# eezkni/UEGAN

Hardware: AMD Instinct MI355X
Metric: train imgs/sec @512px bs=16 on 1/2/4/8 MI355X; infer ms/img (higher is better)
Workload: dtype bf16; 1 GPU; FiveK-shaped 512x512 batch=16/GPU, full G/D/VGG train step (trainer.py:77-119), conv_dim=32, seeded stand-in VGG19; global_batch=16, parallelism=dp1, pool_size=50, collective=none (1 rank), passes=batched (fused.py)

## Files before the change

### include/uegan_hip.h

```cpp
#ifndef UEGAN_HIP_H_
#define UEGAN_HIP_H_

#include <stddef.h>
#include <stdint.h>

#ifdef __cplusplus
extern "C" {
#endif

#define UEGAN_VERSION 105

enum { UEGAN_OK = 0, UEGAN_E_INVALID = -1, UEGAN_E_HIP = -2, UEGAN_E_UNSUPPORTED = -3 };
enum { UEGAN_F32 = 0, UEGAN_BF16 = 1 };
enum { UEGAN_PAD_ZERO = 0, UEGAN_PAD_REFLECT = 1 };
enum { UEGAN_ACT_NONE = 0, UEGAN_ACT_LRELU = 1, UEGAN_ACT_RELU = 2, UEGAN_ACT_TANH = 3,
       UEGAN_ACT_SIGMOID = 4,
       UEGAN_ACT_SWISH = 5, UEGAN_ACT_SELU = 6 };
enum { UEGAN_IMPL_AUTO = 0, UEGAN_IMPL_MFMA = 1, UEGAN_IMPL_DIRECT = 2, UEGAN_IMPL_MFMA_REGSTAGE = 3, UEGAN_IMPL_MFMA_GENERIC = 4 };

typedef void* uegan_stream_t;

int uegan_version(void);
const char* uegan_last_error(void);
int uegan_set_conv_impl(int impl);
enum {
  UEGAN_TUNE_SMALL_GRID = 0,
  UEGAN_TUNE_FOLD_MAX = 1,
  UEGAN_TUNE_HEADS_NO_CG = 2,
  UEGAN_TUNE_WIDE_MIN_GRID = 3,
  UEGAN_TUNE_TALL_MIN_GRID = 4,
  UEGAN_TUNE_TALL_RPW = 5,
  UEGAN_TUNE_TALL_REFLECT = 6,
  UEGAN_TUNE_FLAT_S2 = 7,
  UEGAN_TUNE_TOEP_HEADS = 8,
  UEGAN_TUNE_HEADS_MFMA = 9,
  UEGAN_TUNE_FWD_STATS = 10,
  UEGAN_TUNE_WGRAD_XCD = 11,
  UEGAN_TUNE_VGG_EPI = 12,
  UEGAN_TUNE_GAM_BWD = 13,
  UEGAN_TUNE_COUNT = 14
};
int uegan_set_tuning(int knob, int value, int* previous);
int uegan_selftest_mfma(void* scratch_4096_floats, uegan_stream_t stream);

typedef struct {
  char name[96];
  int64_t launches;
  double total_ms;
  double total_flops;
  double total_bytes;
} uegan_profile_entry;
int uegan_profile_begin(int max_records);
int uegan_profile_end(uegan_profile_entry* out, int max_entries, int* n_entries);

typedef struct {
  int32_t dtype;
  int32_t B, H, W;
  int32_t C1, C2;
  int32_t Ho, Wo, Cout;
  int32_t KH, KW, stride, pad;
  int32_t pad_mode;
  int32_t act;
  int32_t Cin_w, Cout_w;
  int32_t Cin_total;
  int32_t scale_group;
} uegan_conv_desc;

int64_t uegan_packed_k(int64_t k);
int uegan_pack_weights(int dtype, const float* w_oihw, int Cout, int Cin, int KH, int KW, int Cout_pad, int Cin_pad, void* w_ohwi,
                       void* w_ihwo, uegan_stream_t stream);
int uegan_pack_weights_slice(int dtype, const float* w_oihw, int Cout, int Cin, int Cin_total, int KH, int KW, int Cout_pad, int Cin_pad,
                             void* w_ohwi, void* w_ihwo, uegan_stream_t stream);
int uegan_pack_weights_pair(int dtype, const float* w_oihw, int Cout, int Cin, int Cin_total, int KH, int KW, int Cout_pad, int Cin_pad,
                            void* w_ohwi, void* w_ihwo, void* w_ohwi_lo, int dup_cin, uegan_stream_t stream);
typedef struct uegan_pack_entry {
  const float* w_oihw;
  void* w_ohwi;
  void* w_ihwo;
  int64_t start;
  int32_t Cout, Cin, Cin_total, KH, KW, Cout_pad, Cin_pad, Kp, Kp2;
  int32_t flags;
  void* w_ohwi_lo;
} uegan_pack_entry;
int uegan_pack_weights_multi(int dtype, const uegan_pack_entry* table_dev, int n_entries, int64_t total, uegan_stream_t stream);
int uegan_conv2d_fwd(const uegan_conv_desc* d, const void* x1, const void* x2, const void* w_ohwi, const float* bias,
                     const float* scale, void* y, uegan_stream_t stream);
size_t uegan_conv2d_fwd_splitk_workspace_bytes(const uegan_conv_desc* d);
int uegan_conv2d_fwd_splitk(const uegan_conv_desc* d, const void* x1, const void* x2, const void* w_ohwi, const float* bias, const float* scale, void* y,
                            void* workspace, size_t workspace_bytes, uegan_stream_t stream);
size_t uegan_conv2d_fwd_stats_workspace_bytes(const uegan_conv_desc* d);
int uegan_conv2d_fwd_stats(const uegan_conv_desc* d, const void* x1, const void* x2, const void* w_ohwi, const float* bias, const float* scale, void* y,
                           float* mean, float* rstd, float eps, void* workspace, size_t workspace_bytes, int* produced, uegan_stream_t stream);
int uegan_instnorm_apply(int dtype, const void* x, void* y, const float* mean, const float* rstd, int B, int HW, int C, uegan_stream_t stream);
// ... 280 lines not shown
```

### uegan_amd/csrc/conv.hip

```cpp
#include "conv_stream.h"

namespace uegan {

int check_desc(const uegan_conv_desc* d) {
  UEGAN_CHECK_ARG(d != nullptr, "conv desc is null");
  UEGAN_CHECK_ARG(d->dtype == UEGAN_F32 || d->dtype == UEGAN_BF16, "bad dtype %d", d->dtype);
  UEGAN_CHECK_ARG(d->B > 0 && d->H > 0 && d->W > 0 && d->C1 > 0 && d->C2 >= 0 && d->Cout > 0, "bad conv dims");
  UEGAN_CHECK_ARG(d->KH > 0 && d->KW > 0 && d->stride > 0 && d->pad >= 0, "bad conv kernel/stride/pad");
  UEGAN_CHECK_ARG(d->Ho == (d->H + 2 * d->pad - d->KH) / d->stride + 1 && d->Wo == (d->W + 2 * d->pad - d->KW) / d->stride + 1,
                  "Ho/Wo inconsistent with H,W,pad,K,stride");
  if (d->pad_mode == UEGAN_PAD_REFLECT)
    UEGAN_CHECK_ARG(d->pad < d->H && d->pad < d->W, "reflection pad %d must be smaller than the input (%d x %d)", d->pad, d->H, d->W);
  else
    UEGAN_CHECK_ARG(d->pad_mode == UEGAN_PAD_ZERO, "bad pad mode");
  const int epc = d->dtype == UEGAN_F32 ? 4 : 8;
  UEGAN_CHECK_ARG(d->C1 % epc == 0 && d->C2 % epc == 0 && d->Cout % epc == 0,
                  "tensor channel counts must be multiples of %d (one 16-byte chunk): pad them (C1=%d C2=%d Cout=%d)", epc, d->C1, d->C2, d->Cout);
  UEGAN_CHECK_ARG(d->Cin_w >= 0 && d->Cin_w <= d->C1 + d->C2 && d->Cout_w >= 0 && d->Cout_w <= d->Cout, "bad true weight dims");
  UEGAN_CHECK_ARG(d->stride <= 2, "stride > 2 is not built");
  UEGAN_CHECK_ARG(d->scale_group >= 0, "bad scale_group");
  UEGAN_CHECK_ARG(d->Cin_total == 0 || d->Cin_total >= (d->Cin_w ? d->Cin_w : d->C1 + d->C2), "Cin_total must cover the input channels used");
  return UEGAN_OK;
}

ConvGeom fwd_geom(const uegan_conv_desc* d) {
  ConvGeom g;
  g.B = d->B; g.IH = d->H; g.IW = d->W; g.C1 = d->C1; g.C2 = d->C2; g.C = d->C1 + d->C2;
  g.OH = d->Ho; g.OW = d->Wo; g.KH = d->KH; g.KW = d->KW; g.stride = d->stride; g.pad = d->pad; g.pad_mode = d->pad_mode;
  g.mode = 0;
  return g;
}

}

using namespace uegan;

static size_t esize(int dtype) { return dtype == UEGAN_F32 ? 4 : 2; }
static int report_taken(int rc, int* flag, int value) {
  if (rc == UEGAN_OK) *flag = value;
  return rc == 1 ? UEGAN_OK : rc;
}

static void fwd_args(const uegan_conv_desc* d, ConvArgs& a, const void* x1, const void* x2, const void* w_ohwi, const float* bias, const float* scale, void* y) {
  a.g = fwd_geom(d);
  a.in1 = x1; a.in2 = d->C2 ? x2 : x1; a.w = w_ohwi; a.bias = bias; a.scale = scale; a.scale_group = d->scale_group; a.out = y; a.out2 = nullptr; a.n_out1 = 0;
  a.N = d->Cout; a.nbias = cout_w(d); a.Kp = (int)uegan_packed_k((int64_t)d->KH * d->KW * a.g.C); a.act = d->act;
  a.frame = 0; a.fy0 = a.fy1 = a.fx0 = a.fx1 = 0; a.mask = nullptr; a.mask_act = UEGAN_ACT_NONE;
}
static void dgrad_args(const uegan_conv_desc* d, ConvArgs& a, const void* dz, const void* w_ihwo, const float* scale, void* out1, void* out2, bool padded_grid) {
  ConvGeom& g = a.g;
  const int grow = padded_grid ? 2 * d->pad : 0;
  g.B = d->B; g.IH = d->Ho; g.IW = d->Wo; g.C1 = d->Cout; g.C2 = 0; g.C = d->Cout;
  g.OH = d->H + grow; g.OW = d->W + grow; g.KH = d->KH; g.KW = d->KW; g.stride = d->stride;
  g.pad = padded_grid ? 0 : d->pad; g.pad_mode = padded_grid ? UEGAN_PAD_ZERO : d->pad_mode;
  g.mode = 1;
  a.in1 = dz; a.in2 = dz; a.bias = nullptr; a.nbias = 0; a.scale = scale; a.scale_group = d->scale_group; a.act = UEGAN_ACT_NONE;
  a.Kp = (int)uegan_packed_k((int64_t)d->KH * d->KW * d->Cout);
  a.w = w_ihwo; a.N = d->C1 + d->C2;
  a.out = out1; a.out2 = d->C2 ? out2 : nullptr; a.n_out1 = d->C1;
  a.frame = 0; a.fy0 = a.fy1 = a.fx0 = a.fx1 = 0; a.mask = nullptr; a.mask_act = UEGAN_ACT_NONE;
}
static size_t padded_grid_bytes(const uegan_conv_desc* d) {
  return (size_t)d->B * (d->H + 2 * d->pad) * (d->W + 2 * d->pad) * (d->C1 + d->C2) * esize(d->dtype);
}

enum GatherRoute { ROUTE_DIRECT, ROUTE_TOEP, ROUTE_STREAM, ROUTE_MFMA };
static GatherRoute gather_route(const ConvArgs& a, int dtype, ConvStreamPlan& sp) {
  if (g_impl.impl == UEGAN_IMPL_DIRECT) return ROUTE_DIRECT;
  if (g_impl.glds && g_impl.stream && conv_toep_takes(a, dtype)) return ROUTE_TOEP;
  if (g_impl.glds && conv_stream_plan(a, dtype, sp)) return ROUTE_STREAM;
  return ROUTE_MFMA;
}
static bool patch_family(const ConvGeom& g, int dtype) { return g_impl.patch && g_impl.glds && g.KH == g.KW && g.C % (CONV_ROWB / (int)esize(dtype)) == 0; }
static int patch_ks(const ConvGeom& g, int dtype) {
  if (!patch_family(g, dtype)) return 0;
  if (g.stride == 1) {
    if (g.KH == 1 && g.pad == 0) return 1;
    if (g.KH == 3 || g.KH == 5 || g.KH == 7) return g.KH;
  } else if (g.stride == 2 && g.mode == 1) {
    if (g.KH == 3 || g.KH == 5 || g.KH == 7) return (g.KH + 1) / 2;
  }
  return 0;
}
static bool wide_first(const ConvGeom& g, int dtype) { return g.stride == 1 && patch_ks(g, dtype) == 3; }

static bool fwd_on_heads(const uegan_conv_desc* d) { return g_impl.impl != UEGAN_IMPL_DIRECT && g_impl.heads && heads_applicable(d); }
static bool dgrad_on_heads(const uegan_conv_desc* d) { return g_impl.impl != UEGAN_IMPL_DIRECT && g_impl.heads && heads_dgrad_applicable(d); }

static int patch_run(ConvArgs& a, int dtype, hipStream_t s, int ks) {
  if (dtype == UEGAN_F32) return ks <= 3 ? conv_patch_f32_a(a, s, ks) : conv_patch_f32_b(a, s, ks);
  return ks <= 3 ? conv_patch_bf16_a(a, s, ks) : conv_patch_bf16_b(a, s, ks);
}

static int dispatch_conv_gemm(ConvArgs& a, int dtype, hipStream_t s) {
  const ConvGeom& g = a.g;
  if (g_impl.patch && g_impl.glds && g.KH == g.KW && g.stride == 2 && g.mode == 0 && dtype != UEGAN_F32 && g.C == 32) {
    const int rc = conv_s2fwd_run(a, dtype, s);
    if (rc != 1) return rc;
  }
  if (patch_family(g, dtype)) {
    if (wide_first(g, dtype)) {
      int rc = conv_tall_run(a, dtype, s);
      if (rc != 1) return rc;
      rc = conv_wide_run(a, dtype, s);
      if (rc != 1) return rc;
      rc = conv_interior_run(a, dtype, s);
      if (rc != 1 && rc != UEGAN_OK) return rc;
    }
    const int ks = patch_ks(g, dtype);
    if (ks) return patch_run(a, dtype, s, ks);
    const int rc = conv_s2fwd_run(a, dtype, s);
    if (rc != 1) return rc;
  }
  return conv_gemm_run(a, dtype, s);
}

static int run_gather_gemm(ConvArgs& a, int dtype, hipStream_t s, bool* mask_applied = nullptr) {
  if (mask_applied) *mask_applied = false;
  ConvStreamPlan sp;
  switch (gather_route(a, dtype, sp)) {
    case ROUTE_DIRECT: return conv_gemm_run(a, dtype, s);
    case ROUTE_TOEP: return conv_toep_run(a, dtype, s);
    case ROUTE_STREAM:
      if (mask_applied) *mask_applied = a.mask != nullptr;
      {
        ProfScope prof = conv_stream_prof(sp, a.g.mode, s);
        conv_stream_launch(sp, s);
        UEGAN_CHECK_LAUNCH();
      }
      return sp.fixup ? launch_dgrad_images(a, dtype, s, sp.a.xmir != 0) : UEGAN_OK;
    case ROUTE_MFMA: break;
  }
  const int ks = a.g.stride == 1 ? patch_ks(a.g, dtype) : 0;
  if (!(a.g.mode == 1 && ((ks == 3 && a.g.pad_mode != UEGAN_PAD_REFLECT) || ks == 1))) a.mask = nullptr;
  if (mask_applied) *mask_applied = a.mask != nullptr;
  return dispatch_conv_gemm(a, dtype, s);
}

extern "C" int uegan_conv2d_fwd(const uegan_conv_desc* d, const void* x1, const void* x2, const void* w_ohwi, const float* bias,
                                const float* scale, void* y, uegan_stream_t stream) {
  int rc = check_desc(d);
  if (rc) return rc;
  UEGAN_CHECK_ARG(x1 && w_ohwi && y && (d->C2 == 0 || x2), "null pointer");
  ConvArgs a;
  fwd_args(d, a, x1, x2, w_ohwi, bias, scale, y);
  hipStream_t s = (hipStream_t)stream;
  if (fwd_on_heads(d)) {
    ConvStreamPlan sp;
    if (d->act == UEGAN_ACT_SIGMOID || gather_route(a, d->dtype, sp) == ROUTE_MFMA) return heads_fwd(d, x1, w_ohwi, bias, scale, y, s);
  }
// ... 367 lines not shown
```

### uegan_amd/csrc/conv_wide.hip

```cpp
#include "conv_core.h"

namespace uegan {

static __device__ __attribute__((aligned(128))) const unsigned int g_zero_page[512] = {0u};

typedef float f32x16 __attribute__((ext_vector_type(16)));

__device__ __forceinline__ f32x16 mfma32_bf16(u32x4 a, u32x4 b, f32x16 c) {
#ifdef UEGAN_HALF_FP16
  return __builtin_amdgcn_mfma_f32_32x32x16_f16(__builtin_bit_cast(bf16x8_t, a), __builtin_bit_cast(bf16x8_t, b), c, 0, 0, 0);
#else
  return __builtin_amdgcn_mfma_f32_32x32x16_bf16(__builtin_bit_cast(bf16x8_t, a), __builtin_bit_cast(bf16x8_t, b), c, 0, 0, 0);
#endif
}

#define UEGAN_SB() __builtin_amdgcn_sched_barrier(0)

template <int KS, int MODE, bool MASK, int ABL = 0>
__global__ void __launch_bounds__(256, 1) conv_wide_kernel(ConvArgs a) {
  constexpr int TH = 8, TW = 32, BN = 256, NWAVES = 4;
  constexpr int PH = TH + KS - 1, PW = TW + KS - 1;
  constexpr int NPG = (PH * PW + 7) / 8;
  constexpr int NI_P = (NPG + NWAVES - 1) / NWAVES;
  constexpr int PBUFB = NPG * 1024, WHALF = BN * 64, DUMPB = 4096;
// ... 200 lines not shown
    for (int i = 0; i < 4; ++i) {
      f32x4 bv[4];
#pragma unroll
      for (int q = 0; q < 4; ++q) bv[q] = *reinterpret_cast<const f32x4*>(lds_bias + (wn * 128 + i * 32 + 4 * lh + 8 * q) * 4);
#pragma unroll
      for (int j = 0; j < 4; ++j) {
        unsigned char* row = est + (j * 32 + l31) * EROW + i * 64 + 8 * lh;
#pragma unroll
        for (int q = 0; q < 4; ++q) {
          float v[4];
#pragma unroll
          for (int r = 0; r < 4; ++r) {
            const float z = plain ? acc[i][j][4 * q + r] : acc[i][j][4 * q + r] * scale + bv[q][r];
            v[r] = plain ? z : fmaxf(z, slope * z);
          }
          u32x2 pk;
          pk.x = pack_bf16x2(v[0], v[1]);
          pk.y = pack_bf16x2(v[2], v[3]);
          *reinterpret_cast<u32x2*>(row + q * 16) = pk;
        }
      }
    }
  }
  __builtin_amdgcn_wave_barrier();
  {
    const float mslope = a.mask_act == UEGAN_ACT_LRELU ? 0.2f : (a.mask_act == UEGAN_ACT_RELU ? 0.f : 1.f);
    bf16_t* out = static_cast<bf16_t*>(a.out);
    const int nl = n0 + wn * 128 + (lane & 15) * 8;
#pragma unroll 4
    for (int it = 0; it < 32; ++it) {
      const int rr = it * 4 + (lane >> 4);
      const int oy = y0 + wm * 4 + (rr >> 5), ox = x0 + (rr & 31);
      const u32x2 v01 = *reinterpret_cast<const u32x2*>(est + rr * EROW + (lane & 15) * 16);
      const u32x2 v23 = *reinterpret_cast<const u32x2*>(est + rr * EROW + (lane & 15) * 16 + 8);
      u32x4 v = {v01.x, v01.y, v23.x, v23.y};
      if (oy >= g.OH || ox >= g.OW) continue;
      const size_t pix = ((size_t)b * g.OH + oy) * g.OW + ox;
      const size_t o = pix * a.N + nl;
      if (MASK) {
        const u32x4 m = *reinterpret_cast<const u32x4*>(static_cast<const bf16_t*>(a.mask) + o);
#pragma unroll
        for (int d = 0; d < 4; ++d) {
          const float lo = half_lo_to_f32(v[d]) * (half_lo_to_f32(m[d]) > 0.f ? 1.f : mslope);
          const float hi = half_hi_to_f32(v[d]) * (half_hi_to_f32(m[d]) > 0.f ? 1.f : mslope);
          v[d] = pack_bf16x2(lo, hi);
        }
      }
      bf16_t* dst = !a.out2 ? out + o : (nl < a.n_out1 ? out + pix * a.n_out1 + nl : static_cast<bf16_t*>(a.out2) + pix * (a.N - a.n_out1) + (nl - a.n_out1));
      *reinterpret_cast<u32x4*>(dst) = v;
    }
  }
}

template <int NI, int MODE, bool MASK, bool POOL, int RPW = 4, int EPI = 0>
__global__ void __launch_bounds__(256, RPW == 2 ? 2 : 1) conv_tall_kernel(ConvArgs a) {
  static_assert(RPW == 4 || RPW == 2, "rows per wave");
  constexpr bool REFL = MODE == 2;
  static_assert(!REFL || (NI == 4 && !MASK && !POOL), "mirrored images: 128-channel blocks, plain epilogue");
  static_assert(EPI == 0 || (MODE == 1 && MASK && !POOL), "fidelity-loss epilogues: masked data gradients");
  constexpr int KS = 3, TH = 4 * RPW, TW = 32, BN = NI * 32, NWAVES = 4;
  constexpr int PH = TH + KS - 1, PW = TW + KS - 1, NPIX = PH * PW;
  constexpr int NPG = (NPIX + 15) / 16;
  constexpr int NI_P = (NPG + NWAVES - 1) / NWAVES;
  constexpr int PBUFB = NPG * 1024, WSL = BN * 64, NWP = WSL / 1024 / NWAVES;
  constexpr int DUMPB = RPW == 2 ? 1024 : 4096, DUMPW = RPW == 2 ? 0 : 1024;
  constexpr int NT = KS * KS, NLOAD = NWP + 2;
  constexpr bool DGRAD = MODE != 0;
  constexpr int EROW = BN * 2 + 8;
  constexpr int WPIX = RPW * 32;
  constexpr int MAINB = 2 * PBUFB + 4 * WSL, EPIB = NWAVES * WPIX * EROW;
  constexpr int BODYB = MAINB > EPIB ? MAINB : EPIB;
  static_assert(NI_P <= 2 * (NT - 2), "the next chunk's patch pieces must be requested two steps before the chunk ends");
  static_assert((RPW == 2 ? 2 : 1) * (BODYB + DUMPB + BN * 4) <= 160 * 1024, "LDS budget");
  static_assert(NWP >= 1, "at least one weight piece per wave per slice");

  __shared__ __attribute__((aligned(16))) unsigned char lds[BODYB + DUMPB + BN * 4];
  unsigned char* const lds_w = lds + 2 * PBUFB;
  unsigned char* const lds_dump = lds + BODYB;
  unsigned char* const lds_bias = lds_dump + DUMPB;

  const ConvGeom& g = a.g;
  const bf16_t* in1 = static_cast<const bf16_t*>(a.in1);
  const bf16_t* in2 = static_cast<const bf16_t*>(a.in2);
  const bf16_t* w = static_cast<const bf16_t*>(a.w);
  const int tid = threadIdx.x, lane = tid & 63;
  const int wave = __builtin_amdgcn_readfirstlane(tid >> 6);
  const int l31 = lane & 31, lh = lane >> 5;
  int n0 = blockIdx.y * BN;
  int t = blockIdx.x;
  if (a.xcd_map) {
    const int L = blockIdx.x + gridDim.x * blockIdx.y, nby = gridDim.y;
    const int xcd = L & 7, grp = L >> 3;
    n0 = (grp % nby) * BN;
    t = (grp / nby) * 8 + xcd;
  }
  const int tile_x = t % a.ntx; t /= a.ntx;
  const int tile_y = t % a.nty;
  const int b = t / a.nty;
  const int y0 = a.rect_y0 + tile_y * TH, x0 = a.rect_x0 + tile_x * TW;
  const int nchunk = g.C / 32, nchunk1 = g.C1 / 32;
  const int nsteps = nchunk * NT;

  const int q_src = ((lane & 3) ^ ((lane >> 4) & 3)) * 8;
  int ppix[NI_P];
  {
    const int vy0 = DGRAD ? y0 + g.pad - (KS - 1) : y0 - g.pad;
    const int vx0 = DGRAD ? x0 + g.pad - (KS - 1) : x0 - g.pad;
    const bool refl = !DGRAD && g.pad_mode == UEGAN_PAD_REFLECT;
#pragma unroll
    for (int ii = 0; ii < NI_P; ++ii) {
      const int pr = (ii * NWAVES + wave) * 16 + (lane >> 2);
      int pix = -1;
      if (pr < NPIX) {
        const int piy = pr / PW, pix_x = pr - piy * PW;
        int sy = vy0 + piy, sx = vx0 + pix_x;
        if (refl) { sy = reflect_idx(sy, g.IH); sx = reflect_idx(sx, g.IW); }
        if (sy >= 0 && sy < g.IH && sx >= 0 && sx < g.IW) pix = (b * g.IH + sy) * g.IW + sx;
      }
      ppix[ii] = pix;
    }
  }
  const unsigned char* const zero16 = reinterpret_cast<const unsigned char*>(g_zero_page) + (lane & 3) * 16;
  const unsigned char* p_src = zero16;
// ... 42 lines not shown
    if constexpr (REFL) xpr[j] = pr;
  };
  bool r_top[RPW], r_bot[RPW];
  bool e_left = false, e_right = false, c_left = false, c_right = false, edge = false;
  if constexpr (REFL) {
#pragma unroll
    for (int j = 0; j < RPW; ++j) {
      const int y = y0 + wave * RPW + j;
      r_top[j] = y == 1;
      r_bot[j] = y == g.OH - 2;
      edge = edge || r_top[j] || r_bot[j];
    }
    e_left = x0 == 0;
    e_right = x0 <= g.OW - 2 && g.OW - 2 < x0 + TW;
    c_left = x0 + l31 == 1;
    c_right = x0 + l31 == g.OW - 2;
    edge = edge || e_left || e_right;
  } else {
#pragma unroll
    for (int j = 0; j < RPW; ++j) r_top[j] = r_bot[j] = false;
  }
  auto fold1 = [&](u32x4& F, const unsigned char* pb, int ksub, int j, int tap) {
    const int ty = tap / KS, tx = tap - ty * KS;
    const bool ym = ty == 0 ? r_top[j] : (ty == 2 ? r_bot[j] : false);
    const bool xany = tx == 0 ? e_left : (tx == 2 ? e_right : false);
    if (!ym && !xany) return;
    const int dpy = ty == 0 ? -2 * PW : 2 * PW, dpx = tx == 0 ? -2 : 2;
    auto rd = [&](int pr) { return *reinterpret_cast<const u32x4*>(pb + ((pr * 64 + ((lh ^ ((pr >> 2) & 3)) << 4)) ^ (ksub << 5))); };
    if (ym) F = add_frag<bf16_t>(F, rd(xpr[j] + dpy));
    if (xany) {
      const uint32_t m = (tx == 0 ? c_left : c_right) ? 0xffffffffu : 0u;
      u32x4 v = rd(xpr[j] + dpx);
      if (ym) v = add_frag<bf16_t>(v, rd(xpr[j] + dpy + dpx));
      F = add_frag<bf16_t>(F, v & u32x4{m, m, m, m});
    }
  };
  u32x4 wf0[NI], xf0[RPW], wf1[NI], xf1[RPW];
  f32x16 acc[NI][RPW];
#pragma unroll
  for (int i = 0; i < NI; ++i)
#pragma unroll
    for (int j = 0; j < RPW; ++j)
#pragma unroll
      for (int r = 0; r < 16; ++r) acc[i][j][r] = 0.f;
  const bool plain = !a.scale && !a.bias && a.act == UEGAN_ACT_NONE;
  {
    const int n = n0 + wave * 64 + lane;
    const bool live = wave * 64 < BN && !plain && a.bias && n < a.nbias;
    __builtin_amdgcn_global_load_lds((const __attribute__((address_space(1))) void*)(live ? a.bias + n : reinterpret_cast<const float*>(g_zero_page) + lane),
                                     (__attribute__((address_space(3))) void*)(wave * 64 < BN ? lds_bias + wave * 256 : lds_dump + wave * DUMPW), 4, 0, 0);
  }
  const float scale = a.scale ? a.scale[a.scale_group ? b / a.scale_group : 0] : 1.f;

#pragma unroll
  for (int ii = 0; ii < NI_P; ++ii) { patch_piece_prepare(ii, 0, true); patch_piece_issue(); }
#pragma unroll
  for (int h = 0; h < 3; ++h) {
    stage_w_prepare();
#pragma unroll
    for (int i = 0; i < NWP; ++i) stage_w_piece(i);
  }
  wait_vmcnt<NWP>();
  raw_barrier();
#pragma unroll
  for (int j = 0; j < RPW; ++j) set_xad(0, j);
#pragma unroll
  for (int i = 0; i < NI; ++i) wf0[i] = *reinterpret_cast<const u32x4*>(lds_w + wad[i]);
#pragma unroll
  for (int j = 0; j < RPW; ++j) xf0[j] = *reinterpret_cast<const u32x4*>(lds + xad[j]);

#define MF(W, X, i, j) acc[i][j] = mfma32_bf16(W[i], X[j], acc[i][j]); UEGAN_SB();
#define LDW(F, slot, ksub, i) F[i] = *reinterpret_cast<const u32x4*>((slot) + (wad[i] ^ ((ksub) << 5)));
#define LDX(F, pb, ksub, j) F[j] = *reinterpret_cast<const u32x4*>((pb) + (xad[j] ^ ((ksub) << 5)));
#define FOLDX(F, pb, ksub, tapv)                                                           \
  if constexpr (REFL) {                                                                    \
    if (edge) {                                                                            \
      _Pragma("unroll") for (int jf = 0; jf < RPW; ++jf) fold1(F[jf], pb, ksub, jf, tapv); \
    }                                                                                      \
  }
  FOLDX(xf0, lds, 0, 0)
  for (int chunk = 0; chunk < nchunk; ++chunk) {
    const unsigned char* pcur = lds + (chunk & 1) * PBUFB;
    const bool more = chunk + 1 < nchunk;
#pragma unroll
    for (int tap = 0; tap < NT; ++tap) {
      const int step = chunk * NT + tap;
      const unsigned char* ws = lds_w + (step & 3) * WSL;
      const unsigned char* wnext = lds_w + ((step + 1) & 3) * WSL;
      const unsigned char* pnext = tap + 1 == NT ? lds + ((chunk + 1) & 1) * PBUFB : pcur;
      const int ntap = tap + 1 == NT ? 0 : tap + 1;
      UEGAN_SB();
      if constexpr (RPW == 2 && NI == 2) {
        MF(wf0, xf0, 0, 0) LDW(wf1, ws, 1, 0) LDW(wf1, ws, 1, 1) UEGAN_SB();
        MF(wf0, xf0, 0, 1) LDX(xf1, pcur, 1, 0) LDX(xf1, pcur, 1, 1) UEGAN_SB();
        MF(wf0, xf0, 1, 0) stage_w_prepare(); stage_w_piece(0); UEGAN_SB();
        if (2 * tap < NI_P) {
          MF(wf0, xf0, 1, 1) patch_piece_prepare(2 * tap, chunk + 1, more); patch_piece_issue(); patch_piece_prepare(2 * tap + 1, chunk + 1, more); patch_piece_issue(); UEGAN_SB();
        } else {
          MF(wf0, xf0, 1, 1)
        }
        MF(wf1, xf1, 0, 0) set_xad(ntap, 0); set_xad(ntap, 1); UEGAN_SB();
        MF(wf1, xf1, 0, 1) LDW(wf0, wnext, 0, 0) LDW(wf0, wnext, 0, 1) UEGAN_SB();
        MF(wf1, xf1, 1, 0) LDX(xf0, pnext, 0, 0) LDX(xf0, pnext, 0, 1) UEGAN_SB();
        MF(wf1, xf1, 1, 1)
      } else if constexpr (RPW == 2) {
        MF(wf0, xf0, 0, 0) LDW(wf1, ws, 1, 0) LDW(wf1, ws, 1, 1) UEGAN_SB();
// ... 11 lines not shown
        MF(wf1, xf1, 1, 1) LDX(xf0, pnext, 0, 0) LDX(xf0, pnext, 0, 1) UEGAN_SB();
        MF(wf1, xf1, 2, 0) MF(wf1, xf1, 2, 1) MF(wf1, xf1, 3, 0) MF(wf1, xf1, 3, 1)
        FOLDX(xf0, pnext, 0, ntap)
      } else if constexpr (NI == 4) {
        MF(wf0, xf0, 0, 0) stage_w_prepare(); UEGAN_SB();
        MF(wf0, xf0, 0, 1) stage_w_piece(0); UEGAN_SB();
        MF(wf0, xf0, 0, 2) stage_w_piece(1); UEGAN_SB();
        MF(wf0, xf0, 0, 3) patch_piece_prepare(2 * tap, chunk + 1, more); UEGAN_SB();
        MF(wf0, xf0, 1, 0) patch_piece_issue(); UEGAN_SB();
        MF(wf0, xf0, 1, 1) patch_piece_prepare(2 * tap + 1, chunk + 1, more); UEGAN_SB();
        MF(wf0, xf0, 1, 2) patch_piece_issue(); UEGAN_SB();
        MF(wf0, xf0, 1, 3) LDW(wf1, ws, 1, 0) LDW(wf1, ws, 1, 1) UEGAN_SB();
        MF(wf0, xf0, 2, 0) LDW(wf1, ws, 1, 2) LDW(wf1, ws, 1, 3) UEGAN_SB();
        MF(wf0, xf0, 2, 1) LDX(xf1, pcur, 1, 0) LDX(xf1, pcur, 1, 1) UEGAN_SB();
        MF(wf0, xf0, 2, 2) LDX(xf1, pcur, 1, 2) LDX(xf1, pcur, 1, 3) UEGAN_SB();
        MF(wf0, xf0, 2, 3) MF(wf0, xf0, 3, 0) MF(wf0, xf0, 3, 1) MF(wf0, xf0, 3, 2) MF(wf0, xf0, 3, 3)
        FOLDX(xf1, pcur, 1, tap)
        MF(wf1, xf1, 0, 0) set_xad(ntap, 0); UEGAN_SB();
        MF(wf1, xf1, 0, 1) set_xad(ntap, 1); UEGAN_SB();
        MF(wf1, xf1, 0, 2) set_xad(ntap, 2); UEGAN_SB();
        MF(wf1, xf1, 0, 3) set_xad(ntap, 3); UEGAN_SB();
        MF(wf1, xf1, 1, 0) LDW(wf0, wnext, 0, 0) LDW(wf0, wnext, 0, 1) UEGAN_SB();
        MF(wf1, xf1, 1, 1) LDW(wf0, wnext, 0, 2) LDW(wf0, wnext, 0, 3) UEGAN_SB();
        MF(wf1, xf1, 1, 2) LDX(xf0, pnext, 0, 0) LDX(xf0, pnext, 0, 1) UEGAN_SB();
        MF(wf1, xf1, 1, 3) LDX(xf0, pnext, 0, 2) LDX(xf0, pnext, 0, 3) UEGAN_SB();
        MF(wf1, xf1, 2, 0) MF(wf1, xf1, 2, 1) MF(wf1, xf1, 2, 2) MF(wf1, xf1, 2, 3)
        MF(wf1, xf1, 3, 0) MF(wf1, xf1, 3, 1) MF(wf1, xf1, 3, 2) MF(wf1, xf1, 3, 3)
        FOLDX(xf0, pnext, 0, ntap)
      } else {
        static_assert(NI == 2 || NI == 4, "channel fragments per wave");
        MF(wf0, xf0, 0, 0) LDW(wf1, ws, 1, 0) LDW(wf1, ws, 1, 1) UEGAN_SB();
        MF(wf0, xf0, 0, 1) LDX(xf1, pcur, 1, 0) LDX(xf1, pcur, 1, 1) UEGAN_SB();
        MF(wf0, xf0, 0, 2) LDX(xf1, pcur, 1, 2) LDX(xf1, pcur, 1, 3) UEGAN_SB();
        MF(wf0, xf0, 0, 3) stage_w_prepare(); UEGAN_SB();
        MF(wf0, xf0, 1, 0) stage_w_piece(0); UEGAN_SB();
        MF(wf0, xf0, 1, 1) patch_piece_prepare(2 * tap, chunk + 1, more); UEGAN_SB();
        MF(wf0, xf0, 1, 2) patch_piece_issue(); patch_piece_prepare(2 * tap + 1, chunk + 1, more); UEGAN_SB();
        MF(wf0, xf0, 1, 3) patch_piece_issue(); UEGAN_SB();
        MF(wf1, xf1, 0, 0) set_xad(ntap, 0); set_xad(ntap, 1); UEGAN_SB();
        MF(wf1, xf1, 0, 1) set_xad(ntap, 2); set_xad(ntap, 3); LDW(wf0, wnext, 0, 0) LDW(wf0, wnext, 0, 1) UEGAN_SB();
        MF(wf1, xf1, 0, 2) LDX(xf0, pnext, 0, 0) LDX(xf0, pnext, 0, 1) UEGAN_SB();
        MF(wf1, xf1, 0, 3) LDX(xf0, pnext, 0, 2) LDX(xf0, pnext, 0, 3) UEGAN_SB();
        MF(wf1, xf1, 1, 0) MF(wf1, xf1, 1, 1) MF(wf1, xf1, 1, 2) MF(wf1, xf1, 1, 3)
      }
      if (RPW == 2 && NI == 2 && 2 * tap >= NI_P) wait_vmcnt<NWP>();
      else wait_vmcnt<NLOAD>();
      raw_barrier();
    }
  }
#undef MF
#undef LDW
#undef LDX
#undef FOLDX
  wait_vmcnt<0>();

  unsigned char* const est = lds + wave * (WPIX * EROW);
  float tst[EPI == 1 ? 32 : 1], ttot[EPI == 1 ? 24 : 1], tgs = 1.f;
  if constexpr (EPI == 1) {
    const size_t bc = (size_t)g.B * a.N, o0 = (size_t)b * a.N + n0 + (lane % (BN / 8)) * 8;
#pragma unroll
    for (int q = 0; q < 8; ++q) {
      const f32x4 v = *reinterpret_cast<const f32x4*>(a.epi_st + (q >> 1) * bc + o0 + 4 * (q & 1));
#pragma unroll
      for (int e = 0; e < 4; ++e) tst[4 * q + e] = v[e];
    }
#pragma unroll
    for (int q = 0; q < 6; ++q) {
      const f32x4 v = *reinterpret_cast<const f32x4*>(a.epi_tot + o0 * 3 + 4 * q);
#pragma unroll
      for (int e = 0; e < 4; ++e) ttot[4 * q + e] = v[e];
    }
    if (a.epi_gscale) tgs = *a.epi_gscale;
  }
  {
    const float slope = a.act == UEGAN_ACT_LRELU ? 0.2f : (a.act == UEGAN_ACT_RELU ? 0.f : 1.f);
#pragma unroll
    for (int i = 0; i < NI; ++i) {
      f32x4 bv[4];
#pragma unroll
      for (int q = 0; q < 4; ++q) bv[q] = *reinterpret_cast<const f32x4*>(lds_bias + (i * 32 + 4 * lh + 8 * q) * 4);
#pragma unroll
      for (int j = 0; j < RPW; ++j) {
        unsigned char* row = est + (j * 32 + l31) * EROW + i * 64 + 8 * lh;
#pragma unroll
        for (int q = 0; q < 4; ++q) {
          float v[4];
#pragma unroll
          for (int r = 0; r < 4; ++r) {
            const float z = plain ? acc[i][j][4 * q + r] : acc[i][j][4 * q + r] * scale + bv[q][r];
            v[r] = plain ? z : fmaxf(z, slope * z);
          }
          u32x2 pk;
          pk.x = pack_bf16x2(v[0], v[1]);
          pk.y = pack_bf16x2(v[2], v[3]);
          *reinterpret_cast<u32x2*>(row + q * 16) = pk;
        }
      }
    }
  }
  __builtin_amdgcn_wave_barrier();
  {
    constexpr int LPP = BN / 8;
    constexpr int PPI = 64 / LPP;
    const float mslope = a.mask_act == UEGAN_ACT_LRELU ? 0.2f : (a.mask_act == UEGAN_ACT_RELU ? 0.f : 1.f);
    bf16_t* out = static_cast<bf16_t*>(a.out);
    const int lc = lane % LPP, nl = n0 + lc * 8;
// ... 78 lines not shown
            for (int d = 0; d < 4; ++d) {
              const float lo = half_lo_to_f32(vv[d]), hi = half_hi_to_f32(vv[d]);
              if (lo > m[2 * d]) { m[2 * d] = lo; arg[2 * d] = dy * 2 + dx; }
              if (hi > m[2 * d + 1]) { m[2 * d + 1] = hi; arg[2 * d + 1] = dy * 2 + dx; }
            }
          }
        if (py >= PH2 || px >= PW2) continue;
        const size_t po = (((size_t)b * PH2 + py) * PW2 + px) * a.N + nl;
        u32x4 o4 = {pack_bf16x2(m[0], m[1]), pack_bf16x2(m[2], m[3]), pack_bf16x2(m[4], m[5]), pack_bf16x2(m[6], m[7])};
        *reinterpret_cast<u32x4*>(pout + po) = o4;
        if (a.pool_idx && b < a.n_idx) {
          const u32x2 a8 = {arg[0] | (arg[1] << 8) | (arg[2] << 16) | (arg[3] << 24), arg[4] | (arg[5] << 8) | (arg[6] << 16) | (arg[7] << 24)};
          *reinterpret_cast<u32x2*>(static_cast<unsigned char*>(a.pool_idx) + po) = a8;
        }
      }
    }
  }
}

int conv_tall_run(ConvArgs& a, int dtype, hipStream_t s, bool interior) {
  const ConvGeom& g = a.g;
  const int min_grid = g_tuning[UEGAN_TUNE_TALL_MIN_GRID];
  if (min_grid < 0) return 1;
  if (dtype != UEGAN_BF16 || g.stride != 1 || g.KH != 3 || g.KW != 3 || a.frame != 0) return 1;
  if (g.C1 % 32 || g.C2 % 32 || g.C > 1024 || (a.N != 64 && a.N % 128) || g.OW < 32 || g.OH < 16) return 1;
  const bool refl = !interior && g.mode == 1 && g.pad_mode == UEGAN_PAD_REFLECT && g.pad == 1 && !g.C2 && !a.mask && a.N % 128 == 0 &&
                    (!a.out2 || a.n_out1 % 8 == 0) && g.OH >= 4 && g.OW >= 4 && g_tuning[UEGAN_TUNE_TALL_REFLECT] != 0;
  if (!interior && !refl && (a.out2 || (g.mode == 1 && (g.C2 || (g.pad_mode == UEGAN_PAD_REFLECT && g.pad != 0))))) return 1;
  if (interior && (g.mode != 1 || g.C2 || a.mask || (a.out2 && a.n_out1 % 8))) return 1;
  auto simple = [](int act) { return act == UEGAN_ACT_NONE || act == UEGAN_ACT_LRELU || act == UEGAN_ACT_RELU; };
  if (!simple(a.act) || (a.mask && !simple(a.mask_act))) return 1;
  if (a.epi && (interior || refl || g.mode != 1 || !a.mask || a.mask_act != UEGAN_ACT_RELU || a.out2 || g.C2)) return 1;
  const int rpw_knob = g_tuning[UEGAN_TUNE_TALL_RPW];
  bool rpw2 = rpw_knob == 2 || (rpw_knob != 4 && g.C < 512);
  const int nb_n = a.N == 64 ? 1 : a.N / 128;
  {
    const int ntx = interior ? (a.rect_x1 - a.rect_x0) / 32 : (g.OW + 31) / 32;
    const int nty16 = interior ? (a.rect_y1 - a.rect_y0) / 16 : (g.OH + 15) / 16, nty8 = interior ? (a.rect_y1 - a.rect_y0) / 8 : (g.OH + 7) / 8;
    if (g.B * nty16 * ntx * nb_n < min_grid) {
      if (rpw_knob == 4 || g.B * nty8 * ntx * nb_n < min_grid) return 1;
      rpw2 = true;
    }
  }
  const int th = rpw2 ? 8 : 16;
  a.nty = interior ? (a.rect_y1 - a.rect_y0) / th : (g.OH + th - 1) / th;
  a.ntx = interior ? (a.rect_x1 - a.rect_x0) / 32 : (g.OW + 31) / 32;
  const int gm = g.B * a.nty * a.ntx;
  const bool pool = a.pool_out && g.mode == 0 && !a.mask && g.OH % 2 == 0 && g.OW % 2 == 0;
  const double rows = interior ? (double)g.B * (a.rect_y1 - a.rect_y0) * (a.rect_x1 - a.rect_x0) : (g.mode == 0 ? (double)g.B * g.OH * g.OW : (double)g.B * g.IH * g.IW);
  ProfScope prof(prof_key(7, true, a.N == 64 ? 64 : 128, 3, refl ? 2 : g.mode, 16, !pool), 2.0 * rows * a.N * (double)(9 * g.C), s,
                 2.0 * (rows * a.N + (interior ? rows : (double)g.B * g.IH * g.IW) * g.C));
  const dim3 grid(gm, a.N == 64 ? 1 : a.N / 128), block(256);
  a.xcd_map = (grid.y > 1 && gm % 8 == 0) ? 1 : 0;
#define UEGAN_TALL(NI, RPW)                                                                                          \
  do {                                                                                                               \
    if (g.mode == 0 && pool) hipLaunchKernelGGL((conv_tall_kernel<NI, 0, false, true, RPW>), grid, block, 0, s, a);  \
    else if (g.mode == 0) hipLaunchKernelGGL((conv_tall_kernel<NI, 0, false, false, RPW>), grid, block, 0, s, a);    \
    else if (a.mask && a.epi == 1) hipLaunchKernelGGL((conv_tall_kernel<NI, 1, true, false, RPW, 1>), grid, block, 0, s, a); \
    else if (a.mask && a.epi == 2) hipLaunchKernelGGL((conv_tall_kernel<NI, 1, true, false, RPW, 2>), grid, block, 0, s, a); \
    else if (a.mask) hipLaunchKernelGGL((conv_tall_kernel<NI, 1, true, false, RPW>), grid, block, 0, s, a);          \
    else hipLaunchKernelGGL((conv_tall_kernel<NI, 1, false, false, RPW>), grid, block, 0, s, a);                     \
  } while (0)
  if (refl) {
    if (rpw2) hipLaunchKernelGGL((conv_tall_kernel<4, 2, false, false, 2>), grid, block, 0, s, a);
    else hipLaunchKernelGGL((conv_tall_kernel<4, 2, false, false, 4>), grid, block, 0, s, a);
  }
  else if (a.N == 64) { if (rpw2) UEGAN_TALL(2, 2); else UEGAN_TALL(2, 4); }
  else if (rpw2) UEGAN_TALL(4, 2);
  else UEGAN_TALL(4, 4);
#undef UEGAN_TALL
  if (g.mode == 0 && pool) a.pool_done = 1;
  UEGAN_CHECK_LAUNCH();
  return UEGAN_OK;
}

int conv_wide_run(ConvArgs& a, int dtype, hipStream_t s, bool interior) {
  const ConvGeom& g = a.g;
  const int min_grid = g_tuning[UEGAN_TUNE_WIDE_MIN_GRID];
  if (min_grid < 0) return 1;
  if (dtype != UEGAN_BF16 || g.stride != 1 || g.KH != 3 || g.KW != 3 || a.frame != 0) return 1;
  if (g.C % 64 || g.C > 1024 || g.C2 || a.N % 256 || g.OW < 32 || g.OH < 8) return 1;
  if (!interior && (a.out2 || (g.mode == 1 && g.pad_mode == UEGAN_PAD_REFLECT && g.pad != 0))) return 1;
  if (interior && (g.mode != 1 || a.mask || (a.out2 && a.n_out1 % 8))) return 1;
  auto simple = [](int act) { return act == UEGAN_ACT_NONE || act == UEGAN_ACT_LRELU || act == UEGAN_ACT_RELU; };
  if (!simple(a.act) || (a.mask && !simple(a.mask_act))) return 1;
  a.nty = interior ? (a.rect_y1 - a.rect_y0) / 8 : (g.OH + 7) / 8;
  a.ntx = interior ? (a.rect_x1 - a.rect_x0) / 32 : (g.OW + 31) / 32;
  const int gm = g.B * a.nty * a.ntx;
  if (gm * (a.N / 256) < min_grid) return 1;
  const double rows = interior ? (double)g.B * (a.rect_y1 - a.rect_y0) * (a.rect_x1 - a.rect_x0) : (g.mode == 0 ? (double)g.B * g.OH * g.OW : (double)g.B * g.IH * g.IW);
  ProfScope prof(prof_key(7, true, 256, 3, g.mode, 8, true), 2.0 * rows * a.N * (double)(9 * g.C), s,
                 2.0 * (rows * a.N + (interior ? rows : (double)g.B * g.IH * g.IW) * g.C));
  const dim3 grid(gm, a.N / 256), block(256);
  const int nby = a.N / 256;
  a.xcd_map = (nby > 1 && gm % 8 == 0) ? 1 : 0;
#ifdef UEGAN_TOOLS_BUILD
  const int abl = g_abl_wide;
  if (g.mode == 0 && abl == 1) hipLaunchKernelGGL((conv_wide_kernel<3, 0, false, 1>), grid, block, 0, s, a);
  else if (g.mode == 0 && abl == 2) hipLaunchKernelGGL((conv_wide_kernel<3, 0, false, 2>), grid, block, 0, s, a);
  else if (g.mode == 0 && abl == 3) hipLaunchKernelGGL((conv_wide_kernel<3, 0, false, 3>), grid, block, 0, s, a);
  else if (g.mode == 0 && abl == 4) hipLaunchKernelGGL((conv_wide_kernel<3, 0, false, 7>), grid, block, 0, s, a);
  else
#endif
  if (g.mode == 0) hipLaunchKernelGGL((conv_wide_kernel<3, 0, false>), grid, block, 0, s, a);
  else if (a.mask) hipLaunchKernelGGL((conv_wide_kernel<3, 1, true>), grid, block, 0, s, a);
  else hipLaunchKernelGGL((conv_wide_kernel<3, 1, false>), grid, block, 0, s, a);
  UEGAN_CHECK_LAUNCH();
  return UEGAN_OK;
}

int conv_interior_run(ConvArgs& a, int dtype, hipStream_t s) {
  const ConvGeom& g = a.g;
  if (dtype != UEGAN_BF16 || g.mode != 1 || g.stride != 1 || g.KH != 3 || g.KW != 3 || g.pad_mode != UEGAN_PAD_REFLECT || g.pad != 1 || a.frame != 0 || a.mask)
    return 1;
  const int y0 = 16, y1 = (g.OH - 1 - g.pad) / 16 * 16, x0 = 16, x1 = 16 + (g.OW - 1 - g.pad - 16) / 32 * 32;
  if (y1 <= y0 || x1 <= x0 || 2LL * (y1 - y0) * (x1 - x0) < (long long)g.OH * g.OW) return 1;
  a.rect_y0 = y0; a.rect_y1 = y1; a.rect_x0 = x0; a.rect_x1 = x1;
  int rc = conv_tall_run(a, dtype, s, true);
  if (rc == 1) rc = conv_wide_run(a, dtype, s, true);
  if (rc != UEGAN_OK) { a.rect_y0 = a.rect_y1 = a.rect_x0 = a.rect_x1 = 0; return rc; }
  a.border_only = 1;
  return UEGAN_OK;
// ... 4 lines not shown
```

### uegan_amd/csrc/runtime.hip

```cpp
#include "conv_core.h"

#include <stdarg.h>

namespace uegan {

static thread_local char g_err[512] = "";

void set_error(const char* fmt, ...) {
  va_list ap;
  va_start(ap, fmt);
  vsnprintf(g_err, sizeof(g_err), fmt, ap);
  va_end(ap);
}

ConvImpl g_impl = {UEGAN_IMPL_AUTO, true, true, true, true, true};
int g_tuning[UEGAN_TUNE_COUNT] = {256, -1, 0, 192, 192, 0, 1, 1, 1, 1, 1, 1, 1, 1};
int g_abl_stream = 0, g_abl_wide = 0;
#ifdef UEGAN_TOOLS_BUILD
extern "C" int uegan_tools_set_ablation(int stream_wgrad_bits, int wide_variant) {
  g_abl_stream = stream_wgrad_bits;
  g_abl_wide = wide_variant;
  return UEGAN_OK;
}
#endif

bool g_prof_on = false;
std::vector<ProfRecord> g_prof_records;
std::vector<std::pair<hipEvent_t, hipEvent_t>> g_prof_pool;
size_t g_prof_used = 0;

__global__ void selftest_mfma_kernel(float* out) {
  const int lane = threadIdx.x & 63;
  f32x4 acc = {0.f, 0.f, 0.f, 0.f};
  const int ai = lane & 15, ak = lane >> 4;
  acc = mfma_f32(ai == ak ? 1.f : 0.f, 100.f * (lane >> 4) + (lane & 15), acc);
  for (int r = 0; r < 4; ++r) out[lane * 4 + r] = acc[r];
  __attribute__((aligned(16))) unsigned short av[8];
  __attribute__((aligned(16))) unsigned short bv[8];
  for (int e = 0; e < 8; ++e) {
    const int k = 8 * (lane >> 4) + e;
    av[e] = f32_to_bf16((lane & 15) == k ? 1.f : 0.f);
    bv[e] = f32_to_bf16((float)(k * 8 + (lane & 15)) * 0.5f);
  }
  f32x4 acc2 = {0.f, 0.f, 0.f, 0.f};
  acc2 = mfma_bf16(*reinterpret_cast<u32x4*>(av), *reinterpret_cast<u32x4*>(bv), acc2);
  for (int r = 0; r < 4; ++r) out[256 + lane * 4 + r] = acc2[r];
  typedef float f32x16_t __attribute__((ext_vector_type(16)));
  __attribute__((aligned(16))) unsigned short bk[8];
  for (int e = 0; e < 8; ++e) {
    const int k = 8 * (lane >> 5) + e;
    av[e] = f32_to_bf16((lane & 31) == k ? 1.f : 0.f);
    bk[e] = f32_to_bf16((float)(k + 1));
    bv[e] = f32_to_bf16((float)((lane & 31) + 1));
  }
  f32x16_t z16;
  for (int r = 0; r < 16; ++r) z16[r] = 0.f;
  const bf16x8_t a8 = __builtin_bit_cast(bf16x8_t, *reinterpret_cast<u32x4*>(av));
#ifdef UEGAN_HALF_FP16
  const f32x16_t d1 = __builtin_amdgcn_mfma_f32_32x32x16_f16(a8, __builtin_bit_cast(bf16x8_t, *reinterpret_cast<u32x4*>(bk)), z16, 0, 0, 0);
  const f32x16_t d2 = __builtin_amdgcn_mfma_f32_32x32x16_f16(a8, __builtin_bit_cast(bf16x8_t, *reinterpret_cast<u32x4*>(bv)), z16, 0, 0, 0);
#else
  const f32x16_t d1 = __builtin_amdgcn_mfma_f32_32x32x16_bf16(a8, __builtin_bit_cast(bf16x8_t, *reinterpret_cast<u32x4*>(bk)), z16, 0, 0, 0);
  const f32x16_t d2 = __builtin_amdgcn_mfma_f32_32x32x16_bf16(a8, __builtin_bit_cast(bf16x8_t, *reinterpret_cast<u32x4*>(bv)), z16, 0, 0, 0);
#endif
  for (int r = 0; r < 16; ++r) {
    out[512 + lane * 16 + r] = d1[r];
    out[1536 + lane * 16 + r] = d2[r];
  }
}
// ... 75 lines not shown
```

Before: 510.2 imgs/sec.

## Add double-step pipelined schedule for 64-channel tall conv and route C%64==32 convs to it

Adds a SCHED=1 variant of the tall conv kernel for 64-output-channel, 8-row tiles. It processes two taps per barrier, uses an 8-slice weight ring and interleaves MFMA with LDS loads and global prefetch of weights and patches, so fewer barriers and less load latency are exposed. Stride-1 3x3 bf16 convs whose channel count is 32 mod 64 are also sent to the tall kernel first. A new tuning knob (default 1) enables the schedule. Bit 2 of that knob, which would keep 32-in/64-out convs off the stream path, stays off by default. The cost is more LDS use, since the weight ring doubles, and a complex hand schedule that relies on static asserts to stay correct.

Result: no change. 514.5 imgs/sec, median of 3 (+0.8%).

```diff
diff --git a/include/uegan_hip.h b/include/uegan_hip.h
--- a/include/uegan_hip.h
+++ b/include/uegan_hip.h
@@ -38,7 +38,8 @@
   UEGAN_TUNE_WGRAD_XCD = 11,
   UEGAN_TUNE_VGG_EPI = 12,
   UEGAN_TUNE_GAM_BWD = 13,
-  UEGAN_TUNE_COUNT = 14
+  UEGAN_TUNE_TALL64_STEP = 14,
+  UEGAN_TUNE_COUNT = 15
 };
 int uegan_set_tuning(int knob, int value, int* previous);
 int uegan_selftest_mfma(void* scratch_4096_floats, uegan_stream_t stream);
diff --git a/uegan_amd/csrc/conv.hip b/uegan_amd/csrc/conv.hip
--- a/uegan_amd/csrc/conv.hip
+++ b/uegan_amd/csrc/conv.hip
@@ -68,7 +68,8 @@
 static GatherRoute gather_route(const ConvArgs& a, int dtype, ConvStreamPlan& sp) {
   if (g_impl.impl == UEGAN_IMPL_DIRECT) return ROUTE_DIRECT;
   if (g_impl.glds && g_impl.stream && conv_toep_takes(a, dtype)) return ROUTE_TOEP;
-  if (g_impl.glds && conv_stream_plan(a, dtype, sp)) return ROUTE_STREAM;
+  const bool tall32 = (g_tuning[UEGAN_TUNE_TALL64_STEP] & 2) && a.g.C == 32 && a.N == 64 && a.g.KH == 3 && a.g.KW == 3 && a.g.stride == 1;
+  if (g_impl.glds && !tall32 && conv_stream_plan(a, dtype, sp)) return ROUTE_STREAM;
   return ROUTE_MFMA;
 }
 static bool patch_family(const ConvGeom& g, int dtype) { return g_impl.patch && g_impl.glds && g.KH == g.KW && g.C % (CONV_ROWB / (int)esize(dtype)) == 0; }
@@ -96,6 +97,10 @@
   const ConvGeom& g = a.g;
   if (g_impl.patch && g_impl.glds && g.KH == g.KW && g.stride == 2 && g.mode == 0 && dtype != UEGAN_F32 && g.C == 32) {
     const int rc = conv_s2fwd_run(a, dtype, s);
+    if (rc != 1) return rc;
+  }
+  if (g_impl.patch && g_impl.glds && dtype != UEGAN_F32 && g.stride == 1 && g.KH == 3 && g.KW == 3 && g.C % 64 == 32) {
+    const int rc = conv_tall_run(a, dtype, s);
     if (rc != 1) return rc;
   }
   if (patch_family(g, dtype)) {
diff --git a/uegan_amd/csrc/conv_wide.hip b/uegan_amd/csrc/conv_wide.hip
--- a/uegan_amd/csrc/conv_wide.hip
+++ b/uegan_amd/csrc/conv_wide.hip
@@ -276,9 +276,11 @@
   }
 }
 
-template <int NI, int MODE, bool MASK, bool POOL, int RPW = 4, int EPI = 0>
+template <int V> struct IntC { static constexpr int value = V; };
+template <int NI, int MODE, bool MASK, bool POOL, int RPW = 4, int EPI = 0, int SCHED = 0>
 __global__ void __launch_bounds__(256, RPW == 2 ? 2 : 1) conv_tall_kernel(ConvArgs a) {
   static_assert(RPW == 4 || RPW == 2, "rows per wave");
+  static_assert(SCHED == 0 || (SCHED == 1 && NI == 2 && RPW == 2 && MODE != 2), "double step: 64-channel blocks on 8-row tiles");
   constexpr bool REFL = MODE == 2;
   static_assert(!REFL || (NI == 4 && !MASK && !POOL), "mirrored images: 128-channel blocks, plain epilogue");
   static_assert(EPI == 0 || (MODE == 1 && MASK && !POOL), "fidelity-loss epilogues: masked data gradients");
@@ -292,7 +294,8 @@
   constexpr bool DGRAD = MODE != 0;
   constexpr int EROW = BN * 2 + 8;
   constexpr int WPIX = RPW * 32;
-  constexpr int MAINB = 2 * PBUFB + 4 * WSL, EPIB = NWAVES * WPIX * EROW;
+  constexpr int NRING = SCHED == 1 ? 8 : 4;
+  constexpr int MAINB = 2 * PBUFB + NRING * WSL, EPIB = NWAVES * WPIX * EROW;
   constexpr int BODYB = MAINB > EPIB ? MAINB : EPIB;
   static_assert(NI_P <= 2 * (NT - 2), "the next chunk's patch pieces must be requested two steps before the chunk ends");
   static_assert((RPW == 2 ? 2 : 1) * (BODYB + DUMPB + BN * 4) <= 160 * 1024, "LDS budget");
@@ -441,6 +444,140 @@
   }
   const float scale = a.scale ? a.scale[a.scale_group ? b / a.scale_group : 0] : 1.f;
 
+  if constexpr (SCHED == 1) {
+    constexpr int NPD = 3, XK = NT / 2, NPK = (NI_P + NPD - 1) / NPD;
+    static_assert(NI_P <= NPD * (NT - 3 - XK), "chunk c+2's patch pieces: requested after the crossing double step, landed before the last barrier but one of the period");
+    static_assert(NPK <= XK - 1, "chunk c+1's patch pieces must have landed at the barrier in front of the crossing double step");
+    static_assert(NRING == 8 && NWP == 1, "two slices in use, two visible, two landing, two being overwritten; one weight piece per wave per slice");
+    constexpr int DSB = 2 * WSL, RINGM = NRING * WSL - 1;
+    const unsigned char* pptr[NI_P];
+    auto patch_rebuild = [&](int chunk) {
+      const bool first = chunk < nchunk1;
+      const bf16_t* base = first ? in1 : in2;
+      const int cs = first ? g.C1 : g.C2, c0 = (first ? chunk : chunk - nchunk1) * 32 + q_src;
+#pragma unroll
+      for (int ii = 0; ii < NI_P; ++ii)
+        pptr[ii] = (chunk < nchunk && ppix[ii] >= 0) ? reinterpret_cast<const unsigned char*>(base + ((size_t)ppix[ii] * cs + c0)) : zero16;
+    };
+    auto patch_advance = [&](int chunk) {
+      if (chunk == nchunk1 || chunk >= nchunk) patch_rebuild(chunk);
+      else {
+#pragma unroll
+        for (int ii = 0; ii < NI_P; ++ii) pptr[ii] += 64;
+      }
+    };
+    auto patch_piece = [&](int pidx, int buf, bool live) {
+      const int rg = pidx * NWAVES + wave;
+      glds16(pptr[pidx], (live && rg < NPG) ? lds + buf * PBUFB + rg * 1024 : lds_dump);
+    };
+    const uint32_t wofs = (uint32_t)((n0 + wave * 16 + (lane >> 2)) * a.Kp + q_src) * 2u;
+    const unsigned char* const wfirst = reinterpret_cast<const unsigned char*>(w);
+    const unsigned char* wchunk = wfirst;
+    const int wtapb = g.C * 2;
+    int dslot = 0;
+    auto weight_piece = [&](int c0, int j, int half) {
+      const bool live = c0 + j / NT < nchunk;
+      const unsigned char* src = live ? wchunk + ((j / NT) * 64 + (j % NT) * wtapb) : wfirst;
+      glds16(src + wofs, live ? lds_w + ((dslot + 3 * DSB) & RINGM) + half * WSL + wave * 1024 : lds_dump);
+    };
+    int wa0[NI], wa1[NI], wc0[NI], wc1[NI];
+#pragma unroll
+    for (int i = 0; i < NI; ++i) {
+      wa0[i] = 2 * PBUFB + wad[i];
+      wa1[i] = 2 * PBUFB + (wad[i] ^ 32);
+      wc0[i] = wa0[i];
+      wc1[i] = wa1[i];
+    }
+    int xa0[(RPW + KS - 1) * KS], xa1[(RPW + KS - 1) * KS];
+#pragma unroll
+    for (int r = 0; r < RPW + KS - 1; ++r)
+#pragma unroll
+      for (int c = 0; c < KS; ++c) {
+        const int pr = xbase + r * PW + c;
+        xa0[r * KS + c] = pr * 64 + ((lh ^ ((pr >> 2) & 3)) << 4);
+        xa1[r * KS + c] = xa0[r * KS + c] ^ 32;
+      }
+    patch_rebuild(0);
+#pragma unroll
+    for (int ii = 0; ii < NI_P; ++ii) patch_piece(ii, 0, true);
+    dslot = -3 * DSB;
+#pragma unroll
+    for (int h = 0; h < 3; ++h) {
+      weight_piece(0, 2 * h, 0);
+      weight_piece(0, 2 * h + 1, 1);
+      dslot += DSB;
+    }
+    wait_vmcnt<2>();
+    raw_barrier();
+#define MF(W, X, i, j) acc[i][j] = mfma32_bf16(W[i], X[j], acc[i][j]); UEGAN_SB();
+#define XI(tapv, j) (((j) + (DGRAD ? KS - 1 - (tapv) / KS : (tapv) / KS)) * KS + (DGRAD ? KS - 1 - (tapv) % KS : (tapv) % KS))
+#define LDW2(F, A, off) F[0] = *reinterpret_cast<const u32x4*>(lds + A[0] + (off)); F[1] = *reinterpret_cast<const u32x4*>(lds + A[1] + (off));
+#define LDX2(F, A, buf, tapv)                                                        \
+  F[0] = *reinterpret_cast<const u32x4*>(lds + (buf) * PBUFB + A[XI(tapv, 0)]);      \
+  F[1] = *reinterpret_cast<const u32x4*>(lds + (buf) * PBUFB + A[XI(tapv, 1)]);
+    LDW2(wf0, wc0, 0)
+    LDX2(xf0, xa0, 0, 0)
+    auto dstep = [&](auto kc, auto tailc, int c0) __attribute__((always_inline)) {
+      constexpr int K = decltype(kc)::value, TAIL = decltype(tailc)::value;
+      constexpr int JA = 2 * K, JB = 2 * K + 1, JN = 2 * K + 2;
+      constexpr int TA = JA % NT, TB = JB % NT, TN = JN % NT;
+      constexpr int BA = (JA / NT) & 1, BB = (JB / NT) & 1, BQ = (JN / NT) & 1;
+      constexpr bool P1 = TAIL == 0 && K < NPK, P2 = TAIL == 0 && K > XK && K <= XK + NPK;
+      constexpr int PI0 = (P1 ? K : K - XK - 1) * NPD, PB = P1 ? 1 : 0;
+      const bool plive = P1 || c0 + 2 < nchunk;
+      UEGAN_SB();
+      MF(wf0, xf0, 0, 0) LDW2(wf1, wc1, 0) UEGAN_SB();
+      MF(wf0, xf0, 0, 1) LDX2(xf1, xa1, BA, TA) UEGAN_SB();
+      if constexpr (TAIL == 2) {
+        MF(wf0, xf0, 1, 0) MF(wf0, xf0, 1, 1)
+        MF(wf1, xf1, 0, 0) MF(wf1, xf1, 0, 1) MF(wf1, xf1, 1, 0) MF(wf1, xf1, 1, 1)
+        wait_vmcnt<0>();
+      } else {
+        MF(wf0, xf0, 1, 0) weight_piece(c0, JA + 6, 0); UEGAN_SB();
+        if constexpr (P1 || P2) {
+          if constexpr (K == 0 || K == XK + 1) patch_advance(c0 + (P1 ? 1 : 2));
+          MF(wf0, xf0, 1, 1) patch_piece(PI0, PB, plive); UEGAN_SB();
+        } else {
+          MF(wf0, xf0, 1, 1)
+        }
+        MF(wf1, xf1, 0, 0) LDW2(wf0, wc0, WSL) UEGAN_SB();
+        MF(wf1, xf1, 0, 1) LDX2(xf0, xa0, BB, TB) UEGAN_SB();
+        const int dnext = (dslot + DSB) & RINGM;
+        if constexpr (P1 || P2) {
+          MF(wf1, xf1, 1, 0) if (PI0 + 1 < NI_P) patch_piece(PI0 + 1, PB, plive); wc0[0] = wa0[0] + dnext; wc0[1] = wa0[1] + dnext; UEGAN_SB();
+          MF(wf1, xf1, 1, 1) if (PI0 + 2 < NI_P) patch_piece(PI0 + 2, PB, plive); UEGAN_SB();
+        } else {
+          MF(wf1, xf1, 1, 0) wc0[0] = wa0[0] + dnext; wc0[1] = wa0[1] + dnext; UEGAN_SB();
+          MF(wf1, xf1, 1, 1)
+        }
+        MF(wf0, xf0, 0, 0) LDW2(wf1, wc1, WSL) UEGAN_SB();
+        MF(wf0, xf0, 0, 1) LDX2(xf1, xa1, BB, TB) UEGAN_SB();
+        MF(wf0, xf0, 1, 0) weight_piece(c0, JB + 6, 1); UEGAN_SB();
+        MF(wf0, xf0, 1, 1) wc1[0] = wa1[0] + dnext; wc1[1] = wa1[1] + dnext; dslot = dnext; UEGAN_SB();
+        MF(wf1, xf1, 0, 0) LDW2(wf0, wc0, 0) UEGAN_SB();
+        MF(wf1, xf1, 0, 1) LDX2(xf0, xa0, BQ, TN) UEGAN_SB();
+        MF(wf1, xf1, 1, 0) MF(wf1, xf1, 1, 1)
+        if constexpr (P1 || P2) wait_vmcnt<2 + (NI_P - PI0 < NPD ? NI_P - PI0 : NPD)>();
+        else wait_vmcnt<2>();
+      }
+      raw_barrier();
+    };
+    int c0 = 0;
+    for (; c0 + 1 < nchunk; c0 += 2) {
+      dstep(IntC<0>{}, IntC<0>{}, c0); dstep(IntC<1>{}, IntC<0>{}, c0); dstep(IntC<2>{}, IntC<0>{}, c0);
+      dstep(IntC<3>{}, IntC<0>{}, c0); dstep(IntC<4>{}, IntC<0>{}, c0); dstep(IntC<5>{}, IntC<0>{}, c0);
+      dstep(IntC<6>{}, IntC<0>{}, c0); dstep(IntC<7>{}, IntC<0>{}, c0); dstep(IntC<8>{}, IntC<0>{}, c0);
+      wchunk += 128;
+    }
+    if (c0 < nchunk) {
+      dstep(IntC<0>{}, IntC<1>{}, c0); dstep(IntC<1>{}, IntC<1>{}, c0); dstep(IntC<2>{}, IntC<1>{}, c0);
+      dstep(IntC<3>{}, IntC<1>{}, c0); dstep(IntC<4>{}, IntC<2>{}, c0);
+    }
+#undef MF
+#undef XI
+#undef LDW2
+#undef LDX2
+  } else {
 #pragma unroll
   for (int ii = 0; ii < NI_P; ++ii) { patch_piece_prepare(ii, 0, true); patch_piece_issue(); }
 #pragma unroll
@@ -558,6 +695,7 @@
 #undef LDW
 #undef LDX
 #undef FOLDX
+  }
   wait_vmcnt<0>();
 
   unsigned char* const est = lds + wave * (WPIX * EROW);
@@ -742,22 +880,23 @@
                  2.0 * (rows * a.N + (interior ? rows : (double)g.B * g.IH * g.IW) * g.C));
   const dim3 grid(gm, a.N == 64 ? 1 : a.N / 128), block(256);
   a.xcd_map = (grid.y > 1 && gm % 8 == 0) ? 1 : 0;
-#define UEGAN_TALL(NI, RPW)                                                                                          \
-  do {                                                                                                               \
-    if (g.mode == 0 && pool) hipLaunchKernelGGL((conv_tall_kernel<NI, 0, false, true, RPW>), grid, block, 0, s, a);  \
-    else if (g.mode == 0) hipLaunchKernelGGL((conv_tall_kernel<NI, 0, false, false, RPW>), grid, block, 0, s, a);    \
-    else if (a.mask && a.epi == 1) hipLaunchKernelGGL((conv_tall_kernel<NI, 1, true, false, RPW, 1>), grid, block, 0, s, a); \
-    else if (a.mask && a.epi == 2) hipLaunchKernelGGL((conv_tall_kernel<NI, 1, true, false, RPW, 2>), grid, block, 0, s, a); \
-    else if (a.mask) hipLaunchKernelGGL((conv_tall_kernel<NI, 1, true, false, RPW>), grid, block, 0, s, a);          \
-    else hipLaunchKernelGGL((conv_tall_kernel<NI, 1, false, false, RPW>), grid, block, 0, s, a);                     \
+#define UEGAN_TALL(NI, RPW, SCHED)                                                                                                  \
+  do {                                                                                                                              \
+    if (g.mode == 0 && pool) hipLaunchKernelGGL((conv_tall_kernel<NI, 0, false, true, RPW, 0, SCHED>), grid, block, 0, s, a);       \
+    else if (g.mode == 0) hipLaunchKernelGGL((conv_tall_kernel<NI, 0, false, false, RPW, 0, SCHED>), grid, block, 0, s, a);         \
+    else if (a.mask && a.epi == 1) hipLaunchKernelGGL((conv_tall_kernel<NI, 1, true, false, RPW, 1, SCHED>), grid, block, 0, s, a); \
+    else if (a.mask && a.epi == 2) hipLaunchKernelGGL((conv_tall_kernel<NI, 1, true, false, RPW, 2, SCHED>), grid, block, 0, s, a); \
+    else if (a.mask) hipLaunchKernelGGL((conv_tall_kernel<NI, 1, true, false, RPW, 0, SCHED>), grid, block, 0, s, a);               \
+    else hipLaunchKernelGGL((conv_tall_kernel<NI, 1, false, false, RPW, 0, SCHED>), grid, block, 0, s, a);                          \
   } while (0)
   if (refl) {
     if (rpw2) hipLaunchKernelGGL((conv_tall_kernel<4, 2, false, false, 2>), grid, block, 0, s, a);
     else hipLaunchKernelGGL((conv_tall_kernel<4, 2, false, false, 4>), grid, block, 0, s, a);
   }
-  else if (a.N == 64) { if (rpw2) UEGAN_TALL(2, 2); else UEGAN_TALL(2, 4); }
-  else if (rpw2) UEGAN_TALL(4, 2);
-  else UEGAN_TALL(4, 4);
+  else if (a.N == 64 && rpw2 && (g_tuning[UEGAN_TUNE_TALL64_STEP] & 1)) UEGAN_TALL(2, 2, 1);
+  else if (a.N == 64) { if (rpw2) UEGAN_TALL(2, 2, 0); else UEGAN_TALL(2, 4, 0); }
+  else if (rpw2) UEGAN_TALL(4, 2, 0);
+  else UEGAN_TALL(4, 4, 0);
 #undef UEGAN_TALL
   if (g.mode == 0 && pool) a.pool_done = 1;
   UEGAN_CHECK_LAUNCH();
diff --git a/uegan_amd/csrc/runtime.hip b/uegan_amd/csrc/runtime.hip
--- a/uegan_amd/csrc/runtime.hip
+++ b/uegan_amd/csrc/runtime.hip
@@ -14,7 +14,7 @@
 }
 
 ConvImpl g_impl = {UEGAN_IMPL_AUTO, true, true, true, true, true};
-int g_tuning[UEGAN_TUNE_COUNT] = {256, -1, 0, 192, 192, 0, 1, 1, 1, 1, 1, 1, 1, 1};
+int g_tuning[UEGAN_TUNE_COUNT] = {256, -1, 0, 192, 192, 0, 1, 1, 1, 1, 1, 1, 1, 1, 1};
 int g_abl_stream = 0, g_abl_wide = 0;
 #ifdef UEGAN_TOOLS_BUILD
 extern "C" int uegan_tools_set_ablation(int stream_wgrad_bits, int wide_variant) {
```
